# CognitiveAISystems/MAPF-GPT

Measured on AMD Instinct MI355X. Metric: agent-steps/s (env+obs+GPT fwd), higher is better.
Workload: dtype f16x3

## Files before the change

### mapf_gpt_amd/csrc/gpt_kernels_attn_tiles.h

```cpp
#pragma once
#include "gpt_kernels_c256p.h"

namespace mgpt {
namespace fastk {

constexpr int kAttNvb1 = 10, kAttNvb2 = 6;

__device__ unsigned long long g_attn_fallbacks = 0;

template <class T, int NP, int KROW, int VROW, int HS>
__device__ __forceinline__ void attention_exact_tiles(unsigned kr_addr, unsigned vr_addr, const u32x4 (&qf)[2][2], float sc2, f32x16 &o, float &l_run)
{
    float m_run, zero;
    asm volatile("v_mov_b32 %0, 0xff800000\n\tv_mov_b32 %1, 0" : "=v"(m_run), "=v"(zero));
    l_run = zero;
#pragma unroll
    for (int g = 0; g < 16; g++) o[g] = zero;
{
    u32x4 kf[2][2], vf[2][2];
    auto load_k = [&](int kt) {
        const unsigned a = kr_addr + (unsigned)kt * (32 * KROW);
        asm volatile("ds_read_b128 %0, %1" : "=v"(kf[0][0]) : "v"(a) : "memory");
        asm volatile("ds_read_b128 %0, %1 offset:32" : "=v"(kf[1][0]) : "v"(a) : "memory");
        if (NP == 2) {
            asm volatile("ds_read_b128 %0, %1 offset:%2" : "=v"(kf[0][1]) : "v"(a), "n"(kT * KROW) : "memory");
            asm volatile("ds_read_b128 %0, %1 offset:%2" : "=v"(kf[1][1]) : "v"(a), "n"(kT * KROW + 32) : "memory");
        } else { kf[0][1] = kf[0][0]; kf[1][1] = kf[1][0]; }
    };
    load_k(0);
#pragma unroll 1
    for (int kt = 0; kt < kT / 32; kt++) {
        f32x16 sc;
#pragma unroll
        for (int g = 0; g < 16; g++) sc[g] = 0.f;
        asm volatile("s_waitcnt lgkmcnt(0)" ::: "memory");
        __builtin_amdgcn_sched_barrier(0);
#pragma unroll
        for (int ks = 0; ks < 2; ks++) sc = mma<T, NP>(kf[ks], qf[ks], sc);
        __builtin_amdgcn_sched_barrier(0);
        {
            const unsigned a = vr_addr + (unsigned)kt * 64;
            asm volatile("ds_read_b128 %0, %1" : "=v"(vf[0][0]) : "v"(a) : "memory");
            asm volatile("ds_read_b128 %0, %1 offset:32" : "=v"(vf[1][0]) : "v"(a) : "memory");
            if (NP == 2) {
                asm volatile("ds_read_b128 %0, %1 offset:%2" : "=v"(vf[0][1]) : "v"(a), "n"(HS * VROW) : "memory");
                asm volatile("ds_read_b128 %0, %1 offset:%2" : "=v"(vf[1][1]) : "v"(a), "n"(HS * VROW + 32) : "memory");
            } else { vf[0][1] = vf[0][0]; vf[1][1] = vf[1][0]; }
        }
        if (kt + 1 < kT / 32) load_k(kt + 1);
        float mx = sc[0];
#pragma unroll
        for (int g = 1; g < 16; g++) mx = fmaxf(mx, sc[g]);
        mx = other_half_max(mx);
        if (__builtin_amdgcn_ballot_w64(mx > m_run) != 0) {
            const float m_new = fmaxf(m_run, mx);
            const float alpha = __builtin_amdgcn_exp2f((m_run - m_new) * sc2);
            l_run *= alpha;
#pragma unroll
            for (int g = 0; g < 16; g++) o[g] *= alpha;
            m_run = m_new;
        }
        const float nm = -m_run * sc2;
        float psum = 0.f;
#pragma unroll
        for (int g = 0; g < 16; g++) {
            sc[g] = __builtin_amdgcn_exp2f(fmaf(sc[g], sc2, nm));
            psum += sc[g];
        }
        l_run += other_half_sum(psum);
        u32x4 pf[2][2];
#pragma unroll
        for (int mm = 0; mm < 2; mm++) pack_octet<T, NP>(sc, mm, pf[mm]);
        if (kt + 1 < kT / 32) asm volatile("s_waitcnt lgkmcnt(%0)" ::"n"(2 * NP) : "memory");
        else asm volatile("s_waitcnt lgkmcnt(0)" ::: "memory");
        __builtin_amdgcn_sched_barrier(0);
#pragma unroll
        for (int mm = 0; mm < 2; mm++) o = mma<T, NP>(vf[mm], pf[mm], o);
    }
}
}

template <class T, int NP, int KROW, int VROW, int HS>
__device__ __forceinline__ void attention_tiles(unsigned kr_addr, unsigned vr_addr, const u32x4 (&qf)[2][2], int lane, f32x16 &o, float &l_run)
{
    using I0 = std::integral_constant<int, 0>;
    using I1 = std::integral_constant<int, 1>;

    u32x4 kf[2][2], vf[2][2], pf[2][2];
    f32x16 sA, sB;
    constexpr int NM = NP == 2 ? 3 : 1;
    auto amfma = [&](u32x4 a, u32x4 b2, f32x16 c) { return T::mfma(a, b2, c); };
    auto amma = [&](const u32x4 (&a)[2], const u32x4 (&b2)[2], f32x16 c) {
        if (NP == 2) { c = amfma(a[1], b2[0], c); c = amfma(a[0], b2[1], c); }
        return amfma(a[0], b2[0], c);
    };
    auto load_k = [&](auto kt_c) {
        constexpr int off = decltype(kt_c)::value * (32 * KROW);
        asm volatile("ds_read_b128 %0, %1 offset:%2" : "=v"(kf[0][0]) : "v"(kr_addr), "n"(off) : "memory");
        asm volatile("ds_read_b128 %0, %1 offset:%2" : "=v"(kf[1][0]) : "v"(kr_addr), "n"(off + 32) : "memory");
        if (NP == 2) {
            asm volatile("ds_read_b128 %0, %1 offset:%2" : "=v"(kf[0][1]) : "v"(kr_addr), "n"(off + kT * KROW) : "memory");
            asm volatile("ds_read_b128 %0, %1 offset:%2" : "=v"(kf[1][1]) : "v"(kr_addr), "n"(off + kT * KROW + 32) : "memory");
        } else { kf[0][1] = kf[0][0]; kf[1][1] = kf[1][0]; }
    };
    auto load_v = [&](auto kt_c, auto mm_c) {
        constexpr int off = decltype(kt_c)::value * 64 + decltype(mm_c)::value * 32, mm = decltype(mm_c)::value;
        asm volatile("ds_read_b128 %0, %1 offset:%2" : "=v"(vf[mm][0]) : "v"(vr_addr), "n"(off) : "memory");
        if (NP == 2) asm volatile("ds_read_b128 %0, %1 offset:%2" : "=v"(vf[mm][1]) : "v"(vr_addr), "n"(off + HS * VROW) : "memory");
        else vf[mm][1] = vf[mm][0];
    };
    auto lgkm = [&](auto n_c) {
        asm volatile("s_waitcnt lgkmcnt(%0)" ::"n"(decltype(n_c)::value) : "memory");
        __builtin_amdgcn_sched_barrier(0);
    };
    auto place = [&](auto nmf_c, auto nv_c) {
#pragma unroll
        for (int n = 0; n < decltype(nmf_c)::value; n++) {
            __builtin_amdgcn_sched_group_barrier(0x008, 1, 0);
            __builtin_amdgcn_sched_group_barrier(0x002, decltype(nv_c)::value, 0);
        }
        __builtin_amdgcn_sched_group_barrier(0x002, 64, 0);
        __builtin_amdgcn_sched_barrier(0);
    };
    using LK = std::integral_constant<int, 2 * NP>;
    using LV = std::integral_constant<int, NP>;
    load_k(I0{});
    lgkm(I0{});
#pragma unroll
    for (int g = 0; g < 16; g++) sA[g] = 0.f;
#pragma unroll
    for (int ks = 0; ks < 2; ks++) sA = amma(kf[ks], qf[ks], sA);
    __builtin_amdgcn_sched_barrier(0);
    load_k(I1{});
    f32x16 nmb;
    {
        float mx = sA[0];
#pragma unroll
        for (int g = 1; g < 16; g++) mx = fmaxf(mx, sA[g]);
        const float nm = -other_half_max(mx);
#pragma unroll
        for (int g = 0; g < 16; g++) { nmb[g] = nm; sA[g] += nm; }
    }
    float l_part = 0.f;
    auto tile = [&](auto kt_c, f32x16 &cur, f32x16 &nxt) {
        constexpr int kt = decltype(kt_c)::value;
        constexpr bool FIRSTT = kt == 0, LASTT = kt == kT / 32 - 1, HAS2 = kt + 2 < kT / 32;
        if constexpr (!FIRSTT) {
            lgkm(std::integral_constant<int, LASTT ? 0 : LK::value>{});
            o = amma(vf[1], pf[1], o);
#pragma unroll
            for (int g = 0; g < 4; g++) {
                cur[g] = __builtin_amdgcn_exp2f(cur[g]);
                l_part += cur[g];
            }
            place(std::integral_constant<int, NM>{}, std::integral_constant<int, 4>{});
            asm volatile("" : "+v"(o));
        }
        load_v(kt_c, I0{});
        if constexpr (!LASTT) {
            lgkm(LV{});
            nxt = amma(kf[0], qf[0], nmb);
            nxt = amma(kf[1], qf[1], nxt);
        }
#pragma unroll
        for (int g = FIRSTT ? 0 : 4; g < 16; g++) {
            cur[g] = __builtin_amdgcn_exp2f(cur[g]);
            l_part += cur[g];
        }
        pack_octet<T, NP>(cur, 0, pf[0]);
        place(std::integral_constant<int, LASTT ? 0 : 2 * NM>{}, std::integral_constant<int, kAttNvb1>{});
        if constexpr (!LASTT) asm volatile("" : "+v"(nxt));
        load_v(kt_c, I1{});
        lgkm(LV{});
        if constexpr (FIRSTT) {
#pragma unroll
            for (int g = 0; g < 16; g++) o[g] = 0.f;
        }
        o = amma(vf[0], pf[0], o);
        pack_octet<T, NP>(cur, 1, pf[1]);
        place(std::integral_constant<int, NM>{}, std::integral_constant<int, kAttNvb2>{});
        asm volatile("" : "+v"(o));
        if constexpr (HAS2) load_k(std::integral_constant<int, HAS2 ? kt + 2 : 0>{});
    };
    using K0 = std::integral_constant<int, 0>; using K1 = std::integral_constant<int, 1>; using K2 = std::integral_constant<int, 2>; using K3 = std::integral_constant<int, 3>;
    using K4 = std::integral_constant<int, 4>; using K5 = std::integral_constant<int, 5>; using K6 = std::integral_constant<int, 6>; using K7 = std::integral_constant<int, 7>;
    static_assert(kT / 32 == 8, "eight key tiles");
    tile(K0{}, sA, sB); tile(K1{}, sB, sA); tile(K2{}, sA, sB); tile(K3{}, sB, sA);
    tile(K4{}, sA, sB); tile(K5{}, sB, sA); tile(K6{}, sA, sB); tile(K7{}, sB, sA);
    lgkm(I0{});
    o = amma(vf[1], pf[1], o);
    __builtin_amdgcn_sched_barrier(0);
    l_run = other_half_sum(l_part);
    if (__builtin_amdgcn_ballot_w64(!(l_part < 60000.0f)) != 0) {
        if (lane == 0) atomicAdd(&g_attn_fallbacks, 1ull);
        attention_exact_tiles<T, NP, KROW, VROW, HS>(kr_addr, vr_addr, qf, 1.0f, o, l_run);
    }
}

}
}
```

### mapf_gpt_amd/csrc/gpt_kernels_c256b.h

```cpp
#pragma once
#include "gpt_kernels_c256p.h"
#include "gpt_kernels_attn_tiles.h"

namespace mgpt {
namespace fastk {

constexpr int kA256oProjSteps = 16;
constexpr int kA256oPeriod = 8 * kA256StepsPerHead + kA256oProjSteps;


template <class T, int NP>
__global__ __launch_bounds__(256) void pack_attn256q_kernel(const float *__restrict__ w_attn, const float *__restrict__ gain,
                                                            const float *__restrict__ w_proj, uint16_t *__restrict__ out,
                                                            float scale_a, float scale_p)
{
    constexpr int C = 256, NH = 8, QKV = NH * kA256StepsPerHead;
    const int64_t gid = (int64_t)blockIdx.x * 256 + threadIdx.x;
    if (gid >= (int64_t)kA256oPeriod * 8 * 64) return;
    const int lane = (int)(gid & 63), ms = (int)((gid >> 6) & 7), G = (int)(gid >> 9);
    const int rho = lane & 15, qk = lane >> 4;
    float v[8];
    if (G < QKV) {
        const int head = G / kA256StepsPerHead, st = G - head * kA256StepsPerHead;
        int which, kb, dim;
        if (st < 4) {
            const int cc = 4 * st + (ms >> 1), ug = ms & 1, rq = rho >> 2;
            kb = cc >> 1; which = cc & 1;
            const int blk = which == 0 ? 2 * (rq & 1) + (rq >> 1) : rq;
            dim = 8 * blk + 4 * ug + (rho & 3);
        } else { which = 2; kb = 4 * (st - 4) + (ms >> 1); dim = 16 * (ms & 1) + rho; }
        const float *row = w_attn + (size_t)(which * C + head * 32 + dim) * C;
#pragma unroll
        for (int e = 0; e < 8; e++) {
            const int col = 32 * kb + 8 * qk + e;
            v[e] = row[col] * gain[col] * scale_a;
        }
    } else {
        const int s = G - QKV, tt = s >> 2, j = s & 3;
        const int cc = 4 * j + (ms >> 1), kb = cc >> 1, fgl = 2 * (cc & 1) + (ms & 1);
        const float *row = w_proj + (size_t)(64 * tt + 16 * fgl + rho) * C;
#pragma unroll
        for (int e = 0; e < 8; e++) {
            const int col = 32 * kb + (e & 3) + 8 * (2 * (qk & 1) + (e >> 2)) + 4 * (qk >> 1);
            v[e] = row[col] * scale_p;
        }
    }
    u32x2 h0, l0, h1, l1;
    split4<T, NP>(v, h0, l0);
    split4<T, NP>(v + 4, h1, l1);
    u32x4 hi, lo;
    hi[0] = h0[0]; hi[1] = h0[1]; hi[2] = h1[0]; hi[3] = h1[1];
    lo[0] = l0[0]; lo[1] = l0[1]; lo[2] = l1[0]; lo[3] = l1[1];
    uint16_t *dst = out + (((size_t)G * 8 + ms) * NP) * 512 + (size_t)lane * 8;
    *reinterpret_cast<u32x4 *>(dst) = hi;
    if (NP == 2) *reinterpret_cast<u32x4 *>(dst + 512) = lo;
}

template <int NP> constexpr int kL0TabHeadBytes = 192 * NP;
template <int NP> constexpr int kL0TabEntryBytes = 8 * kL0TabHeadBytes<NP>;
template <class T, int NP, bool EMB = false, int TAB = 0>
__global__ __launch_bounds__(512, 2) void attn256q_kernel(float *__restrict__ x, const uint16_t *__restrict__ wstream, float inv_scale,
                                                          float scale_log2e, float inv_proj, unsigned char *__restrict__ spill,
                                                          int n_rows, const unsigned char *__restrict__ tokens = nullptr,
                                                          const float *__restrict__ etab = nullptr, unsigned char *__restrict__ table = nullptr)
{
    static_assert(TAB == 0 || (TAB == 1 && EMB) || (TAB == 2 && !EMB), "table modes");
    constexpr int HB = kL0TabHeadBytes<NP>, ENT = kL0TabEntryBytes<NP>;
    constexpr int C = 256, KS = 16, NH = 8, HS = 32, NW = 8;
    static_assert(NP == 2 || NP == 1, "planes");
    constexpr int MS = 8;
    constexpr int STEP = MS * NP * 1024;
    constexpr int NSLOT = 5;
    constexpr int PW = MS * NP / NW;
    constexpr int KROW = 80, VROW = 528;
    constexpr int NSPILL = 2 * NP;
    constexpr int NYLD = 14 * NP;
    static_assert(PW >= 1, "a wave moves at least one piece per step");
    extern __shared__ __attribute__((aligned(16))) unsigned char smem[];
    const int tid = threadIdx.x, lane = tid & 63;
    const int wave = __builtin_amdgcn_readfirstlane(tid >> 6);
    const int tok0 = wave * 32;
    const unsigned lane16 = (unsigned)lane * 16u;
    const unsigned lds0 = (unsigned)(size_t)smem + lane16;
    const unsigned sK = (unsigned)(size_t)smem + NSLOT * STEP, sV = sK + NP * kT * KROW;
    constexpr int PERIOD = TAB == 2 ? kA256oProjSteps : kA256oPeriod;
    const unsigned char *wbase = reinterpret_cast<const unsigned char *>(wstream) + (size_t)(wave * PW) * 1024 +
                                 (TAB == 2 ? (size_t)(kA256oPeriod - kA256oProjSteps) * STEP : 0);
    unsigned char *sp_wave = spill + ((size_t)blockIdx.x * NW + wave) * (size_t)(14 * NP * 1024);
    const int n_mine = n_rows > (int)blockIdx.x ? (n_rows - 1 - (int)blockIdx.x) / (int)gridDim.x + 1 : 0;
    if (n_mine == 0) return;

    int r_issue = 0;
    int slot_cur = 0, slot_prev = NSLOT - 1;
    unsigned cur_addr = 0, nxt_addr = 0;
    auto issue = [&](int slot) {
        const unsigned char *src = wbase + (size_t)r_issue * STEP;
        unsigned char *dst = smem + (size_t)slot * STEP + (size_t)(wave * PW) * 1024;
#pragma unroll
        for (int i = 0; i < PW; i++) dma_piece(src + lane16, dst, std::integral_constant<int, 0>{}, i);
        r_issue = r_issue + 1 == PERIOD ? 0 : r_issue + 1;
    };
#pragma unroll
    for (int G = 0; G < NSLOT - 1; G++) issue(G);
    auto sync_wait = [&](auto pending_c) {
        vm_wait<decltype(pending_c)::value>();
        __builtin_amdgcn_s_barrier();
    };
    int slot_refill = 0;
    auto sync_issue = [&]() {
        issue(slot_prev);
        const int slot_next = slot_cur + 1 == NSLOT ? 0 : slot_cur + 1;
        cur_addr = lds0 + (unsigned)slot_cur * STEP;
        nxt_addr = lds0 + (unsigned)slot_next * STEP;
        slot_prev = slot_cur;
        slot_cur = slot_next;
    };
    u32x4 wb[2][2][2];
    auto chunk_wait = [&]() {
        asm volatile("s_waitcnt lgkmcnt(0)" ::: "memory");
        __builtin_amdgcn_sched_barrier(0);
    };
    auto chunk_read = [&](auto c_c, auto next_c, auto n_c) {
        constexpr int c = decltype(c_c)::value, n = decltype(n_c)::value;
        if constexpr (n < 2 * NP) {
            constexpr int fr = n / NP, pl = n % NP;
            if constexpr (c < 3) lds_frag(cur_addr, std::integral_constant<int, ((2 * c + 2 + fr) * NP + pl) * 1024>{}, wb[(c + 1) & 1][fr][pl]);
            else if constexpr (decltype(next_c)::value) lds_frag(nxt_addr, std::integral_constant<int, (fr * NP + pl) * 1024>{}, wb[0][fr][pl]);
            if constexpr (NP == 1 && (c < 3 || decltype(next_c)::value)) wb[(c + 1) & 1][fr][1] = wb[(c + 1) & 1][fr][0];
            __builtin_amdgcn_sched_barrier(0);
        }
    };
    using I0 = std::integral_constant<int, 0>;
    using I1 = std::integral_constant<int, 1>;
    using I2 = std::integral_constant<int, 2>;
    using I3 = std::integral_constant<int, 3>;
    auto mma4 = [&](const u32x4 (&w0)[2], const u32x4 (&w1)[2], const u32x4 (&x0)[2], const u32x4 (&x1)[2], f32x16 &blk, auto swap_c, auto first_c, auto &&behind) {
        constexpr bool SW = decltype(swap_c)::value, FIRST = decltype(first_c)::value;
        auto one = [&](const u32x4 &w, const u32x4 &xx, auto s_c) {
            if constexpr (SW) mm16<T>(xx, w, blk, s_c); else mm16<T>(w, xx, blk, s_c);
        };
        auto onez = [&](const u32x4 &w, const u32x4 &xx, auto s_c) {
            if constexpr (!FIRST) one(w, xx, s_c);
            else if constexpr (SW) mm16z<T>(xx, w, blk, s_c);
            else mm16z<T>(w, xx, blk, s_c);
        };
        if (NP == 2) {
            onez(w0[1], x0[0], I0{}); behind(I0{}); onez(w1[1], x0[0], I1{}); behind(I1{}); onez(w0[1], x1[0], I2{}); behind(I2{}); onez(w1[1], x1[0], I3{}); behind(I3{});
            one(w0[0], x0[1], I0{}); behind(std::integral_constant<int, 4>{}); one(w1[0], x0[1], I1{}); behind(std::integral_constant<int, 5>{});
            one(w0[0], x1[1], I2{}); one(w1[0], x1[1], I3{});
            one(w0[0], x0[0], I0{}); one(w1[0], x0[0], I1{}); one(w0[0], x1[0], I2{}); one(w1[0], x1[0], I3{});
        } else {
            onez(w0[0], x0[0], I0{}); behind(I0{}); onez(w1[0], x0[0], I1{}); behind(I1{}); onez(w0[0], x1[0], I2{}); behind(I2{}); onez(w1[0], x1[0], I3{});
        }
    };
    auto chunk_body = [&](auto c_c, auto next_c, auto &&mm) {
        chunk_wait();
        constexpr bool REFILL = false;
        constexpr int N_REFILL = NP == 2 ? 5 : 2, N_LAST = REFILL ? N_REFILL : 2 * NP - 1, NMF = NP == 2 ? 12 : 4;
        mm([&](auto n_c) {
            constexpr int n = decltype(n_c)::value;
            if constexpr (n < 2 * NP) { __builtin_amdgcn_sched_barrier(0); chunk_read(c_c, next_c, n_c); }
            else if constexpr (REFILL && n == N_REFILL) { __builtin_amdgcn_sched_barrier(0); issue(slot_refill); __builtin_amdgcn_sched_barrier(0); }
        });
#pragma unroll
        for (int n = 0; n < NMF - 1 - N_LAST; n++) __builtin_amdgcn_sched_group_barrier(0x008, 1, 0);
        __builtin_amdgcn_sched_barrier(0);
    };
    const float q_units = scale_log2e * inv_scale, k_units = inv_scale;

    u32x4 xn[KS][2];

    f32x16 qa, ka;
    auto step_pair = [&](auto j_c, auto pending_c, auto &&after_barrier, auto next_c) {
        constexpr int j = decltype(j_c)::value;
        sync_wait(pending_c);
        after_barrier();
        sync_issue();
        auto chunk = [&](auto c_c) {
            constexpr int c = decltype(c_c)::value;
            constexpr int cc = 4 * j + c, kb = cc >> 1;
            chunk_body(c_c, next_c, [&](auto &&behind) {
                using F = std::integral_constant<bool, (cc < 2)>;
                if constexpr ((cc & 1) == 0) mma4(wb[c & 1][0], wb[c & 1][1], xn[kb], xn[8 + kb], qa, std::false_type{}, F{}, behind);
                else mma4(wb[c & 1][0], wb[c & 1][1], xn[kb], xn[8 + kb], ka, std::false_type{}, F{}, behind);
            });
            asm volatile("" : "+v"(qa), "+v"(ka));
        };
        chunk(I0{}); chunk(I1{}); chunk(I2{}); chunk(I3{});
    };
    auto nothing = [&]() {};
    asm volatile("s_waitcnt vmcnt(0)" ::: "memory");
    __builtin_amdgcn_s_barrier();
    nxt_addr = lds0;
    using P4 = std::integral_constant<int, PW * (NSLOT - 3)>;
    using P4S = std::integral_constant<int, PW * (NSLOT - 3) + NSPILL>;

#pragma unroll 1
    for (int k = 0; k < n_mine; k++) {
        const int64_t b = (int64_t)blockIdx.x + (int64_t)k * gridDim.x;
        unsigned char *xw = reinterpret_cast<unsigned char *>(x + (b * kT + tok0) * C);
        unsigned ent0 = 0, ent1 = 0;
        if constexpr (TAB == 2) {
            unsigned l16p = lane16;
            asm volatile("" : "+v"(l16p));
            const unsigned char *tk = tokens + b * kT + tok0;
            const unsigned tt_p = (l16p >> 4) & 15u;
            unsigned id0, id1;
            asm volatile("global_load_ubyte %0, %1, %2" : "=v"(id0) : "v"(tt_p), "s"(tk) : "memory");
            asm volatile("global_load_ubyte %0, %1, %2 offset:16" : "=v"(id1) : "v"(tt_p), "s"(tk) : "memory");
            asm volatile("s_waitcnt vmcnt(0)" : "+v"(id0), "+v"(id1) : : "memory");
            ent0 = ((unsigned)tok0 + tt_p) * 67u + id0;
            ent1 = ((unsigned)tok0 + 16u + tt_p) * 67u + id1;
        } else {
            unsigned l16p = lane16;
            asm volatile("" : "+v"(l16p));
            const unsigned xoff_p = (l16p >> 8) * 1024 + ((l16p >> 4) & 15u) * 32;
            f32x4 xr[32];
            if constexpr (EMB) {
                const unsigned char *tk = tokens + b * kT + tok0;
                const unsigned tt_p = (l16p >> 4) & 15u;
                unsigned id0, id1;
                asm volatile("global_load_ubyte %0, %1, %2" : "=v"(id0) : "v"(tt_p), "s"(tk) : "memory");
                asm volatile("global_load_ubyte %0, %1, %2 offset:16" : "=v"(id1) : "v"(tt_p), "s"(tk) : "memory");
                asm volatile("s_waitcnt vmcnt(0)" : "+v"(id0), "+v"(id1) : : "memory");
                const unsigned q32 = (l16p >> 8) * 32u;
                const unsigned ve0 = (((unsigned)tok0 + tt_p) * 67u + id0) * 1024u + q32;
                const unsigned ve1 = (((unsigned)tok0 + 16u + tt_p) * 67u + id1) * 1024u + q32;
                const unsigned char *eb = reinterpret_cast<const unsigned char *>(etab);
#pragma unroll
                for (int i = 0; i < 32; i++) {
                    if (((i >> 1) & 1) == 0)
                        asm volatile("global_load_dwordx4 %0, %1, %2 offset:%3" : "=v"(xr[2 * (i >> 2) + (i & 1)]) : "v"(ve0), "s"(eb), "n"((i >> 2) * 128 + (i & 1) * 16) : "memory");
                    else
                        asm volatile("global_load_dwordx4 %0, %1, %2 offset:%3" : "=v"(xr[2 * (8 + (i >> 2)) + (i & 1)]) : "v"(ve1), "s"(eb), "n"((i >> 2) * 128 + (i & 1) * 16) : "memory");
                }
            } else {
#pragma unroll
            for (int i = 0; i < 32; i++) {
                const unsigned char *xq = xw + (i >> 2) * 4096;
                asm volatile("global_load_dwordx4 %0, %1, %2 offset:%3" : "=v"(xr[2 * (8 * ((i >> 1) & 1) + (i >> 2)) + (i & 1)]) : "v"(xoff_p), "s"(xq), "n"(((i >> 1) & 1) * 512 + (i & 1) * 16) : "memory");
            }
            }
            asm volatile("s_waitcnt vmcnt(0)" : "+v"(xr[0]), "+v"(xr[1]), "+v"(xr[2]), "+v"(xr[3]), "+v"(xr[4]), "+v"(xr[5]), "+v"(xr[6]), "+v"(xr[7]) : : "memory");
            asm volatile("" : "+v"(xr[8]), "+v"(xr[9]), "+v"(xr[10]), "+v"(xr[11]), "+v"(xr[12]), "+v"(xr[13]), "+v"(xr[14]), "+v"(xr[15]));
            asm volatile("" : "+v"(xr[16]), "+v"(xr[17]), "+v"(xr[18]), "+v"(xr[19]), "+v"(xr[20]), "+v"(xr[21]), "+v"(xr[22]), "+v"(xr[23]));
            asm volatile("" : "+v"(xr[24]), "+v"(xr[25]), "+v"(xr[26]), "+v"(xr[27]), "+v"(xr[28]), "+v"(xr[29]), "+v"(xr[30]), "+v"(xr[31]));
            if constexpr (EMB) {
#pragma unroll
                for (int i = 0; i < 32; i++) {
                    const unsigned char *xq = xw + (i >> 2) * 4096;
                    asm volatile("global_store_dwordx4 %0, %1, %2 offset:%3\n\ts_nop 1" ::"v"(xoff_p), "v"(xr[2 * (8 * ((i >> 1) & 1) + (i >> 2)) + (i & 1)]), "s"(xq), "n"(((i >> 1) & 1) * 512 + (i & 1) * 16) : "memory");
                }
            }
            float rstd[2];
#pragma unroll
            for (int tg = 0; tg < 2; tg++) {
                float sm = 0.f;
#pragma unroll
                for (int i = 0; i < 16; i++) sm += (xr[16 * tg + i][0] + xr[16 * tg + i][1]) + (xr[16 * tg + i][2] + xr[16 * tg + i][3]);
                const float mean = permlane_fold4(sm) * (1.0f / (float)C);
                float qv = 0.f;
#pragma unroll
                for (int i = 0; i < 16; i++)
#pragma unroll
                    for (int e = 0; e < 4; e++) { const float d = xr[16 * tg + i][e] - mean; xr[16 * tg + i][e] = d; qv = fmaf(d, d, qv); }
                rstd[tg] = rsqrtf(permlane_fold4(qv) * (1.0f / (float)C) + 1e-5f);
            }
#pragma unroll
            for (int ks = 0; ks < KS; ks++) {
                float v0[4], v1[4];
#pragma unroll
                for (int e = 0; e < 4; e++) { v0[e] = xr[2 * ks][e] * rstd[ks >> 3]; v1[e] = xr[2 * ks + 1][e] * rstd[ks >> 3]; }
                u32x2 h0, l0, h1, l1;
                split4p<T, NP>(v0, h0, l0);
                split4p<T, NP>(v1, h1, l1);
                xn[ks][0][0] = h0[0]; xn[ks][0][1] = h0[1]; xn[ks][0][2] = h1[0]; xn[ks][0][3] = h1[1];
                xn[ks][1][0] = l0[0]; xn[ks][1][1] = l0[1]; xn[ks][1][2] = l1[0]; xn[ks][1][3] = l1[1];
                if ((ks & 1) == 1) __builtin_amdgcn_sched_barrier(0);
            }
        }
        if constexpr (TAB != 2) {
            lds_pair<NP>(nxt_addr, I0{}, wb[0][0]);
            lds_pair<NP>(nxt_addr, I1{}, wb[0][1]);
        }

        auto head = [&](int hd, auto last_c) {
            constexpr bool LASTH = decltype(last_c)::value;
            unsigned l16 = lane16;
            asm volatile("" : "+v"(l16));
            const unsigned rr = (l16 >> 4) & 31u, hh = l16 >> 9;
            const unsigned kr_addr = sK + rr * KROW + hh * 16;
            const unsigned vr_addr = sV + rr * VROW + hh * 16;
            const unsigned tt = (l16 >> 4) & 15u, qq = l16 >> 8;
            const unsigned kw_addr = sK + ((unsigned)tok0 + tt) * KROW + qq * 16;
            const unsigned vw_addr = sV + tt * VROW + (unsigned)wave * 64 + (qq & 1u) * 16 + (qq >> 1) * 8;
            asm volatile("" : "=v"(qa), "=v"(ka));
            step_pair(I0{}, P4S{}, nothing, std::true_type{});
            step_pair(I1{}, P4S{}, nothing, std::true_type{});
            step_pair(I2{}, P4S{}, nothing, std::true_type{});
            step_pair(I3{}, P4{}, nothing, std::true_type{});
            u32x4 qf[2][2];
#pragma unroll
            for (int g = 0; g < 16; g++) { qa[g] *= q_units; ka[g] *= k_units; }
#pragma unroll
            for (int tg = 0; tg < 2; tg++) pack_octet<T, NP>(qa, tg, qf[tg]);
#pragma unroll
            for (int pl = 0; pl < NP; pl++)
#pragma unroll
                for (int wd = 0; wd < 4; wd++) { unsigned a = qf[0][pl][wd], b2 = qf[1][pl][wd]; row_swap(a, b2); qf[0][pl][wd] = a; qf[1][pl][wd] = b2; }
            if (NP == 1) { qf[0][1] = qf[0][0]; qf[1][1] = qf[1][0]; }
            if constexpr (TAB == 1) {
                const unsigned voff = (((unsigned)tok0 + rr) * 67u * ENT) + (unsigned)b * ENT + (unsigned)hd * HB + hh * (32 * NP);
#pragma unroll
                for (int ks = 0; ks < 2; ks++)
#pragma unroll
                    for (int pl = 0; pl < NP; pl++)
                        asm volatile("global_store_dwordx4 %0, %1, %2 offset:%3\n\ts_nop 1" ::"v"(voff), "v"(qf[ks][pl]), "s"(table), "n"((ks * NP + pl) * 16) : "memory");
            }
            {
                u32x4 kp[2][2];
#pragma unroll
                for (int tg = 0; tg < 2; tg++) pack_octet<T, NP>(ka, tg, kp[tg]);
#pragma unroll
                for (int tg = 0; tg < 2; tg++)
#pragma unroll
                    for (int pl = 0; pl < NP; pl++)
                        asm volatile("ds_write_b128 %0, %1 offset:%2" ::"v"(kw_addr), "v"(kp[tg][pl]), "n"(pl * kT * KROW + tg * 16 * KROW) : "memory");
                if constexpr (TAB == 1) {
#pragma unroll
                    for (int tg = 0; tg < 2; tg++) {
                        const unsigned voff = (((unsigned)tok0 + 16u * tg + tt) * 67u * ENT) + (unsigned)b * ENT + (unsigned)hd * HB + 64 * NP + qq * (16 * NP);
#pragma unroll
                        for (int pl = 0; pl < NP; pl++)
                            asm volatile("global_store_dwordx4 %0, %1, %2 offset:%3\n\ts_nop 1" ::"v"(voff), "v"(kp[tg][pl]), "s"(table), "n"(pl * 16) : "memory");
                    }
                }
            }
            f32x16 va;
            auto step_v = [&](auto j_c, auto next_c) {
                constexpr int j = decltype(j_c)::value;
                sync_wait(P4{});
                sync_issue();
                auto chunk = [&](auto c_c) {
                    constexpr int c = decltype(c_c)::value;
                    constexpr int kb = 4 * j + c;
                    chunk_body(c_c, next_c, [&](auto &&behind) { mma4(wb[c & 1][0], wb[c & 1][1], xn[kb], xn[8 + kb], va, std::true_type{}, std::integral_constant<bool, kb == 0>{}, behind); });
                    asm volatile("" : "+v"(va));
                };
                chunk(I0{}); chunk(I1{}); chunk(I2{}); chunk(I3{});
            };
            step_v(I0{}, std::true_type{});
            step_v(I1{}, std::false_type{});
            if constexpr (LASTH) {
#pragma unroll
                for (int hh2 = 0; hh2 < 7; hh2++)
#pragma unroll
                    for (int tg = 0; tg < 2; tg++)
#pragma unroll
                        for (int pl = 0; pl < NP; pl++) {
                            const unsigned char *p = sp_wave + (size_t)hh2 * (size_t)(2 * NP * 1024);
                            asm volatile("global_load_dwordx4 %0, %1, %2 offset:%3" : "=v"(xn[8 * tg + hh2][pl]) : "v"(lane16), "s"(p), "n"((tg * NP + pl) * 1024) : "memory");
                        }
            }
            {
#pragma unroll
                for (int sl = 0; sl < 4; sl++) {
                    u32x2 vp[2];
                    unsigned a0, b0, a1, b1;
                    split2p<T, NP>(va[4 * sl], va[4 * sl + 1], a0, b0);
                    split2p<T, NP>(va[4 * sl + 2], va[4 * sl + 3], a1, b1);
                    vp[0][0] = a0; vp[0][1] = a1; vp[1][0] = b0; vp[1][1] = b1;
#pragma unroll
                    for (int pl = 0; pl < NP; pl++)
                        asm volatile("ds_write_b64 %0, %1 offset:%2" ::"v"(vw_addr), "v"(vp[pl]), "n"(pl * HS * VROW + (sl & 1) * 16 * VROW + (sl >> 1) * 32) : "memory");
                    if constexpr (TAB == 1) {
#pragma unroll
                        for (int i = 0; i < 4; i++) {
                            const unsigned voff = (((unsigned)tok0 + 16u * (sl >> 1) + 4u * qq + i) * 67u * ENT) + (unsigned)b * ENT + (unsigned)hd * HB + 128 * NP +
                                                  (16u * (sl & 1) + tt) * 2u;
#pragma unroll
                            for (int pl = 0; pl < NP; pl++) {
                                if (i & 1) asm volatile("global_store_short_d16_hi %0, %1, %2 offset:%3" ::"v"(voff), "v"(vp[pl][i >> 1]), "s"(table), "n"(pl * 64) : "memory");
                                else asm volatile("global_store_short %0, %1, %2 offset:%3" ::"v"(voff), "v"(vp[pl][i >> 1]), "s"(table), "n"(pl * 64) : "memory");
                            }
                        }
                    }
                }
            }
            if constexpr (TAB == 1) asm volatile("s_waitcnt vmcnt(0)" ::: "memory");
            asm volatile("s_waitcnt lgkmcnt(0)" ::: "memory");
            __builtin_amdgcn_s_barrier();

            f32x16 o;
            float l_run = 0.f;
            attention_tiles<T, NP, KROW, VROW, HS>(kr_addr, vr_addr, qf, lane, o, l_run);
            lds_pair<NP>(nxt_addr, I0{}, wb[0][0]);
            lds_pair<NP>(nxt_addr, I1{}, wb[0][1]);
            {
                const float inv = inv_scale / l_run;
#pragma unroll
                for (int g = 0; g < 16; g++) o[g] *= inv;
#pragma unroll
                for (int g = 0; g < 8; g++) { float a = o[g], b2 = o[8 + g]; asm volatile("s_nop 1\n\tv_permlane16_swap_b32 %0, %1" : "+v"(a), "+v"(b2)); o[g] = a; o[8 + g] = b2; }
                if constexpr (LASTH) {
                    pack_octet<T, NP>(o, 0, xn[7]);
                    pack_octet<T, NP>(o, 1, xn[15]);
                } else {
                    u32x4 yp[2][2];
                    pack_octet<T, NP>(o, 0, yp[0]);
                    pack_octet<T, NP>(o, 1, yp[1]);
                    unsigned char *p = sp_wave + (size_t)hd * (size_t)(2 * NP * 1024);
#pragma unroll
                    for (int kk = 0; kk < 2; kk++)
#pragma unroll
                        for (int pl = 0; pl < NP; pl++)
                            asm volatile("global_store_dwordx4 %0, %1, %2 offset:%3\n\ts_nop 1" ::"v"(lane16), "v"(yp[kk][pl]), "s"(p), "n"((kk * NP + pl) * 1024) : "memory");
                }
            }
        };
        auto head_t = [&](int hd) {
            unsigned l16 = lane16;
            asm volatile("" : "+v"(l16));
            const unsigned rr = (l16 >> 4) & 31u, hh = l16 >> 9;
            const unsigned kr_addr = sK + rr * KROW + hh * 16;
            const unsigned vr_addr = sV + rr * VROW + hh * 16;
            const unsigned tt = (l16 >> 4) & 15u, qq = l16 >> 8;
            const unsigned kw_addr = sK + ((unsigned)tok0 + tt) * KROW + qq * 16;
            const unsigned vt_addr = sV + qq * 8 * VROW + (unsigned)wave * 64 + (((tt >> 2) & 1u) * 8 + ((tt >> 3) & 1u) * 4 + (tt & 3u)) * 2;
            const unsigned hoff = (unsigned)hd * HB;
            const unsigned e0 = ent0 * ENT + hoff, e1 = ent1 * ENT + hoff;
            const unsigned qoff = ((qq & 1u) ? e1 : e0) + hh * (32 * NP);
            u32x4 qf[2][2], kp[2][2], vq[2][2];
#pragma unroll
            for (int ks = 0; ks < 2; ks++)
#pragma unroll
                for (int pl = 0; pl < NP; pl++)
                    asm volatile("global_load_dwordx4 %0, %1, %2 offset:%3" : "=v"(qf[ks][pl]) : "v"(qoff), "s"(table), "n"((ks * NP + pl) * 16) : "memory");
#pragma unroll
            for (int tg = 0; tg < 2; tg++) {
                const unsigned ko = (tg ? e1 : e0) + qq * (16 * NP), vo = (tg ? e1 : e0) + qq * 16;
#pragma unroll
                for (int pl = 0; pl < NP; pl++) {
                    asm volatile("global_load_dwordx4 %0, %1, %2 offset:%3" : "=v"(kp[tg][pl]) : "v"(ko), "s"(table), "n"(64 * NP + pl * 16) : "memory");
                    asm volatile("global_load_dwordx4 %0, %1, %2 offset:%3" : "=v"(vq[tg][pl]) : "v"(vo), "s"(table), "n"(128 * NP + pl * 64) : "memory");
                }
            }
            __builtin_amdgcn_s_barrier();
            if constexpr (NP == 2)
                asm volatile("s_waitcnt vmcnt(0)" : "+v"(qf[0][0]), "+v"(qf[0][1]), "+v"(qf[1][0]), "+v"(qf[1][1]), "+v"(kp[0][0]), "+v"(kp[0][1]), "+v"(kp[1][0]), "+v"(kp[1][1]),
                             "+v"(vq[0][0]), "+v"(vq[0][1]), "+v"(vq[1][0]), "+v"(vq[1][1]) : : "memory");
            else
                asm volatile("s_waitcnt vmcnt(0)" : "+v"(qf[0][0]), "+v"(qf[1][0]), "+v"(kp[0][0]), "+v"(kp[1][0]), "+v"(vq[0][0]), "+v"(vq[1][0]) : : "memory");
            if (NP == 1) { qf[0][1] = qf[0][0]; qf[1][1] = qf[1][0]; }
#pragma unroll
            for (int tg = 0; tg < 2; tg++)
#pragma unroll
                for (int pl = 0; pl < NP; pl++) {
                    asm volatile("ds_write_b128 %0, %1 offset:%2" ::"v"(kw_addr), "v"(kp[tg][pl]), "n"(pl * kT * KROW + tg * 16 * KROW) : "memory");
#pragma unroll
                    for (int j = 0; j < 8; j++) {
                        if (j & 1) asm volatile("ds_write_b16_d16_hi %0, %1 offset:%2" ::"v"(vt_addr), "v"(vq[tg][pl][j >> 1]), "n"(pl * HS * VROW + j * VROW + tg * 32) : "memory");
                        else asm volatile("ds_write_b16 %0, %1 offset:%2" ::"v"(vt_addr), "v"(vq[tg][pl][j >> 1]), "n"(pl * HS * VROW + j * VROW + tg * 32) : "memory");
                    }
                }
            asm volatile("s_waitcnt lgkmcnt(0)" ::: "memory");
            __builtin_amdgcn_s_barrier();
            f32x16 o;
            float l_run = 0.f;
            attention_tiles<T, NP, KROW, VROW, HS>(kr_addr, vr_addr, qf, lane, o, l_run);
            const float inv = inv_scale / l_run;
#pragma unroll
            for (int g = 0; g < 16; g++) o[g] *= inv;
#pragma unroll
            for (int g = 0; g < 8; g++) { float a = o[g], b2 = o[8 + g]; asm volatile("s_nop 1\n\tv_permlane16_swap_b32 %0, %1" : "+v"(a), "+v"(b2)); o[g] = a; o[8 + g] = b2; }
#pragma unroll
            for (int k2 = 0; k2 < 7; k2++)
#pragma unroll
                for (int pl = 0; pl < NP; pl++) { xn[k2][pl] = xn[k2 + 1][pl]; xn[8 + k2][pl] = xn[9 + k2][pl]; }
            pack_octet<T, NP>(o, 0, xn[7]);
            pack_octet<T, NP>(o, 1, xn[15]);
        };
        if constexpr (TAB == 2) {
#pragma unroll 1
            for (int hd = 0; hd < NH; hd++) head_t(hd);
            lds_pair<NP>(nxt_addr, I0{}, wb[0][0]);
            lds_pair<NP>(nxt_addr, I1{}, wb[0][1]);
        } else {
#pragma unroll 1
            for (int hd = 0; hd < NH - 1; hd++) head(hd, std::false_type{});
            head(NH - 1, std::true_type{});
        }

        auto tail = [&](int t, auto first_c, auto last_c) {
            constexpr bool FIRST = decltype(first_c)::value, LASTT = decltype(last_c)::value;
            asm volatile("" : "=v"(qa), "=v"(ka));
            unsigned l16t = lane16;
            asm volatile("" : "+v"(l16t));
            const unsigned xoff_t = (l16t >> 9) * 1024 + ((l16t >> 4) & 15u) * 32 + ((l16t >> 8) & 1u) * 16;
            const unsigned qq_t = l16t >> 8;
            f32x4 xs[4][2];
            unsigned char *xp = xw + (size_t)t * 8192;
            constexpr int OTHERS = 8;
            auto requests = [&]() {
                if constexpr (TAB == 2) {
                    const unsigned r0 = ent0 * (C * 4) + (unsigned)t * 256 + qq_t * 16, r1 = ent1 * (C * 4) + (unsigned)t * 256 + qq_t * 16;
                    const unsigned char *eb = reinterpret_cast<const unsigned char *>(etab);
#pragma unroll
                    for (int fgl = 0; fgl < 4; fgl++) {
                        asm volatile("global_load_dwordx4 %0, %1, %2 offset:%3" : "=v"(xs[fgl][0]) : "v"(r0), "s"(eb), "n"(fgl * 64) : "memory");
                        asm volatile("global_load_dwordx4 %0, %1, %2 offset:%3" : "=v"(xs[fgl][1]) : "v"(r1), "s"(eb), "n"(fgl * 64) : "memory");
                    }
                    return;
                }
#pragma unroll
                for (int fgl = 0; fgl < 4; fgl++)
#pragma unroll
                    for (int tg = 0; tg < 2; tg++)
                        asm volatile("global_load_dwordx4 %0, %1, %2 offset:%3" : "=v"(xs[fgl][tg]) : "v"(xoff_t), "s"(xp + (fgl >> 1) * 4096), "n"((fgl & 1) * 2048 + tg * 512) : "memory");
            };
            step_pair(I0{}, std::integral_constant<int, 2 * PW + (FIRST ? (TAB == 2 ? 0 : NYLD) : 8)>{}, requests, std::true_type{});
            step_pair(I1{}, std::integral_constant<int, 2 * PW + 8 + OTHERS>{}, nothing, std::true_type{});
            step_pair(I2{}, std::integral_constant<int, 2 * PW + 8 + OTHERS>{}, nothing, std::true_type{});
            step_pair(I3{}, P4{}, nothing, std::integral_constant<bool, !LASTT>{});
            asm volatile("s_waitcnt vmcnt(%[n])" : "+v"(xs[0][0]), "+v"(xs[0][1]), "+v"(xs[1][0]), "+v"(xs[1][1]), "+v"(xs[2][0]), "+v"(xs[2][1]), "+v"(xs[3][0]), "+v"(xs[3][1])
                         : [n] "n"(4 * PW) : "memory");
#pragma unroll
            for (int fgl = 0; fgl < 4; fgl++)
#pragma unroll
                for (int tg = 0; tg < 2; tg++) {
                    f32x4 v;
#pragma unroll
                    for (int e = 0; e < 4; e++) v[e] = fmaf((fgl < 2 ? qa : ka)[4 * (2 * tg + (fgl & 1)) + e], inv_proj, xs[fgl][tg][e]);
                    asm volatile("global_store_dwordx4 %0, %1, %2 offset:%3\n\ts_nop 1" ::"v"(xoff_t), "v"(v), "s"(xp + (fgl >> 1) * 4096), "n"((fgl & 1) * 2048 + tg * 512) : "memory");
                }
        };
        {
            asm volatile("s_waitcnt vmcnt(0)" : "+v"(xn[0][0]), "+v"(xn[0][1]), "+v"(xn[1][0]), "+v"(xn[1][1]), "+v"(xn[2][0]), "+v"(xn[2][1]), "+v"(xn[3][0]), "+v"(xn[3][1]),
                         "+v"(xn[4][0]), "+v"(xn[4][1]), "+v"(xn[5][0]), "+v"(xn[5][1]), "+v"(xn[6][0]), "+v"(xn[6][1]) : : "memory");
            asm volatile("" : "+v"(xn[8][0]), "+v"(xn[8][1]), "+v"(xn[9][0]), "+v"(xn[9][1]), "+v"(xn[10][0]), "+v"(xn[10][1]), "+v"(xn[11][0]), "+v"(xn[11][1]),
                         "+v"(xn[12][0]), "+v"(xn[12][1]), "+v"(xn[13][0]), "+v"(xn[13][1]), "+v"(xn[14][0]), "+v"(xn[14][1]));
            asm volatile("" : "+v"(xn[7][0]), "+v"(xn[7][1]), "+v"(xn[15][0]), "+v"(xn[15][1]));
        }
        tail(0, std::true_type{}, std::false_type{});
#pragma unroll 1
        for (int t = 1; t < 3; t++) tail(t, std::false_type{}, std::false_type{});
        tail(3, std::false_type{}, std::true_type{});
    }
    asm volatile("s_waitcnt vmcnt(0)" ::: "memory");
}

}
}
```

Before: 128,300.

## Prefetch next head's Q/K/V table rows during attention via hook and LDS staging

In the TAB==2 path, the next head's K/V table entries are now staged into LDS with global_load_lds right after each head's barrier. The next head's Q fragments are prefetched into registers through a new hook called inside attention_tiles near the final tile. A fallback hook reloads the current Q if the exact-attention path runs. The weight-ring DMA prologue is deferred until the last head and held during the last tail step, with the vmcnt waits adjusted to match. The aim is to hide global-load latency of per-head table reads behind attention compute, at the cost of more complex wait-count bookkeeping and extra LDS staging space.

After: 128,300 (median of 3 runs). No clear change (-0.0%).

```diff
diff --git a/mapf_gpt_amd/csrc/gpt_kernels_attn_tiles.h b/mapf_gpt_amd/csrc/gpt_kernels_attn_tiles.h
--- a/mapf_gpt_amd/csrc/gpt_kernels_attn_tiles.h
+++ b/mapf_gpt_amd/csrc/gpt_kernels_attn_tiles.h
@@ -80,8 +80,12 @@
 }
 }
 
-template <class T, int NP, int KROW, int VROW, int HS>
-__device__ __forceinline__ void attention_tiles(unsigned kr_addr, unsigned vr_addr, const u32x4 (&qf)[2][2], int lane, f32x16 &o, float &l_run)
+struct attn_no_hook {
+    template <class P> __device__ __forceinline__ void operator()(P) const {}
+};
+
+template <class T, int NP, int KROW, int VROW, int HS, class Hook = attn_no_hook>
+__device__ __forceinline__ void attention_tiles(unsigned kr_addr, unsigned vr_addr, const u32x4 (&qf)[2][2], int lane, f32x16 &o, float &l_run, Hook hook = Hook{})
 {
     using I0 = std::integral_constant<int, 0>;
     using I1 = std::integral_constant<int, 1>;
@@ -170,6 +174,7 @@
         pack_octet<T, NP>(cur, 0, pf[0]);
         place(std::integral_constant<int, LASTT ? 0 : 2 * NM>{}, std::integral_constant<int, kAttNvb1>{});
         if constexpr (!LASTT) asm volatile("" : "+v"(nxt));
+        if constexpr (kt == kT / 32 - 2) hook(I0{});
         load_v(kt_c, I1{});
         lgkm(LV{});
         if constexpr (FIRSTT) {
@@ -193,7 +198,9 @@
     l_run = other_half_sum(l_part);
     if (__builtin_amdgcn_ballot_w64(!(l_part < 60000.0f)) != 0) {
         if (lane == 0) atomicAdd(&g_attn_fallbacks, 1ull);
+        hook(I1{});
         attention_exact_tiles<T, NP, KROW, VROW, HS>(kr_addr, vr_addr, qf, 1.0f, o, l_run);
+        hook(std::integral_constant<int, 2>{});
     }
 }
 
diff --git a/mapf_gpt_amd/csrc/gpt_kernels_c256b.h b/mapf_gpt_amd/csrc/gpt_kernels_c256b.h
--- a/mapf_gpt_amd/csrc/gpt_kernels_c256b.h
+++ b/mapf_gpt_amd/csrc/gpt_kernels_c256b.h
@@ -93,15 +93,19 @@
     int r_issue = 0;
     int slot_cur = 0, slot_prev = NSLOT - 1;
     unsigned cur_addr = 0, nxt_addr = 0;
+    bool ring_hold = false;
     auto issue = [&](int slot) {
+        if constexpr (TAB == 2) { if (ring_hold) return; }
         const unsigned char *src = wbase + (size_t)r_issue * STEP;
         unsigned char *dst = smem + (size_t)slot * STEP + (size_t)(wave * PW) * 1024;
 #pragma unroll
         for (int i = 0; i < PW; i++) dma_piece(src + lane16, dst, std::integral_constant<int, 0>{}, i);
         r_issue = r_issue + 1 == PERIOD ? 0 : r_issue + 1;
     };
+    if constexpr (TAB != 2) {
 #pragma unroll
     for (int G = 0; G < NSLOT - 1; G++) issue(G);
+    }
     auto sync_wait = [&](auto pending_c) {
         vm_wait<decltype(pending_c)::value>();
         __builtin_amdgcn_s_barrier();
@@ -211,6 +215,7 @@
             asm volatile("s_waitcnt vmcnt(0)" : "+v"(id0), "+v"(id1) : : "memory");
             ent0 = ((unsigned)tok0 + tt_p) * 67u + id0;
             ent1 = ((unsigned)tok0 + 16u + tt_p) * 67u + id1;
+            asm volatile("" : "+v"(ent0), "+v"(ent1));
         } else {
             unsigned l16p = lane16;
             asm volatile("" : "+v"(l16p));
@@ -418,6 +423,7 @@
                 }
             }
         };
+        u32x4 qf[2][2];
         auto head_t = [&](int hd) {
             unsigned l16 = lane16;
             asm volatile("" : "+v"(l16));
@@ -428,29 +434,49 @@
             const unsigned kw_addr = sK + ((unsigned)tok0 + tt) * KROW + qq * 16;
             const unsigned vt_addr = sV + qq * 8 * VROW + (unsigned)wave * 64 + (((tt >> 2) & 1u) * 8 + ((tt >> 3) & 1u) * 4 + (tt & 3u)) * 2;
             const unsigned hoff = (unsigned)hd * HB;
-            const unsigned e0 = ent0 * ENT + hoff, e1 = ent1 * ENT + hoff;
+            unsigned en0 = ent0, en1 = ent1;
+            asm volatile("" : "+v"(en0), "+v"(en1));
+            const unsigned e0 = en0 * ENT + hoff, e1 = en1 * ENT + hoff;
             const unsigned qoff = ((qq & 1u) ? e1 : e0) + hh * (32 * NP);
-            u32x4 qf[2][2], kp[2][2], vq[2][2];
-#pragma unroll
-            for (int ks = 0; ks < 2; ks++)
-#pragma unroll
-                for (int pl = 0; pl < NP; pl++)
-                    asm volatile("global_load_dwordx4 %0, %1, %2 offset:%3" : "=v"(qf[ks][pl]) : "v"(qoff), "s"(table), "n"((ks * NP + pl) * 16) : "memory");
-#pragma unroll
-            for (int tg = 0; tg < 2; tg++) {
-                const unsigned ko = (tg ? e1 : e0) + qq * (16 * NP), vo = (tg ? e1 : e0) + qq * 16;
-#pragma unroll
-                for (int pl = 0; pl < NP; pl++) {
-                    asm volatile("global_load_dwordx4 %0, %1, %2 offset:%3" : "=v"(kp[tg][pl]) : "v"(ko), "s"(table), "n"(64 * NP + pl * 16) : "memory");
-                    asm volatile("global_load_dwordx4 %0, %1, %2 offset:%3" : "=v"(vq[tg][pl]) : "v"(vo), "s"(table), "n"(128 * NP + pl * 64) : "memory");
-                }
-            }
-            __builtin_amdgcn_s_barrier();
-            if constexpr (NP == 2)
-                asm volatile("s_waitcnt vmcnt(0)" : "+v"(qf[0][0]), "+v"(qf[0][1]), "+v"(qf[1][0]), "+v"(qf[1][1]), "+v"(kp[0][0]), "+v"(kp[0][1]), "+v"(kp[1][0]), "+v"(kp[1][1]),
-                             "+v"(vq[0][0]), "+v"(vq[0][1]), "+v"(vq[1][0]), "+v"(vq[1][1]) : : "memory");
-            else
-                asm volatile("s_waitcnt vmcnt(0)" : "+v"(qf[0][0]), "+v"(qf[1][0]), "+v"(kp[0][0]), "+v"(kp[1][0]), "+v"(vq[0][0]), "+v"(vq[1][0]) : : "memory");
+            u32x4 kp[2][2], vq[2][2];
+            const unsigned st_addr = (unsigned)(size_t)smem + l16 + (unsigned)wave * (4 * NP * 1024);
+            if (hd == 0) {
+#pragma unroll
+                for (int ks = 0; ks < 2; ks++)
+#pragma unroll
+                    for (int pl = 0; pl < NP; pl++)
+                        asm volatile("global_load_dwordx4 %0, %1, %2 offset:%3" : "=v"(qf[ks][pl]) : "v"(qoff), "s"(table), "n"((ks * NP + pl) * 16) : "memory");
+#pragma unroll
+                for (int tg = 0; tg < 2; tg++) {
+                    const unsigned ko = (tg ? e1 : e0) + qq * (16 * NP), vo = (tg ? e1 : e0) + qq * 16;
+#pragma unroll
+                    for (int pl = 0; pl < NP; pl++) {
+                        asm volatile("global_load_dwordx4 %0, %1, %2 offset:%3" : "=v"(kp[tg][pl]) : "v"(ko), "s"(table), "n"(64 * NP + pl * 16) : "memory");
+                        asm volatile("global_load_dwordx4 %0, %1, %2 offset:%3" : "=v"(vq[tg][pl]) : "v"(vo), "s"(table), "n"(128 * NP + pl * 64) : "memory");
+                    }
+                }
+                __builtin_amdgcn_s_barrier();
+                if constexpr (NP == 2)
+                    asm volatile("s_waitcnt vmcnt(0)" : "+v"(qf[0][0]), "+v"(qf[0][1]), "+v"(qf[1][0]), "+v"(qf[1][1]), "+v"(kp[0][0]), "+v"(kp[0][1]), "+v"(kp[1][0]), "+v"(kp[1][1]),
+                                 "+v"(vq[0][0]), "+v"(vq[0][1]), "+v"(vq[1][0]), "+v"(vq[1][1]) : : "memory");
+                else
+                    asm volatile("s_waitcnt vmcnt(0)" : "+v"(qf[0][0]), "+v"(qf[1][0]), "+v"(kp[0][0]), "+v"(kp[1][0]), "+v"(vq[0][0]), "+v"(vq[1][0]) : : "memory");
+            } else {
+                __builtin_amdgcn_s_barrier();
+                if constexpr (NP == 2) asm volatile("s_waitcnt vmcnt(0)" : "+v"(qf[0][0]), "+v"(qf[0][1]), "+v"(qf[1][0]), "+v"(qf[1][1]) : : "memory");
+                else asm volatile("s_waitcnt vmcnt(0)" : "+v"(qf[0][0]), "+v"(qf[1][0]) : : "memory");
+#pragma unroll
+                for (int tg = 0; tg < 2; tg++)
+#pragma unroll
+                    for (int pl = 0; pl < NP; pl++) {
+                        asm volatile("ds_read_b128 %0, %1 offset:%2" : "=v"(kp[tg][pl]) : "v"(st_addr), "n"(2 * (tg * NP + pl) * 1024) : "memory");
+                        asm volatile("ds_read_b128 %0, %1 offset:%2" : "=v"(vq[tg][pl]) : "v"(st_addr), "n"((2 * (tg * NP + pl) + 1) * 1024) : "memory");
+                    }
+                if constexpr (NP == 2)
+                    asm volatile("s_waitcnt lgkmcnt(0)" : "+v"(kp[0][0]), "+v"(kp[0][1]), "+v"(kp[1][0]), "+v"(kp[1][1]), "+v"(vq[0][0]), "+v"(vq[0][1]), "+v"(vq[1][0]), "+v"(vq[1][1]) : : "memory");
+                else
+                    asm volatile("s_waitcnt lgkmcnt(0)" : "+v"(kp[0][0]), "+v"(kp[1][0]), "+v"(vq[0][0]), "+v"(vq[1][0]) : : "memory");
+            }
             if (NP == 1) { qf[0][1] = qf[0][0]; qf[1][1] = qf[1][0]; }
 #pragma unroll
             for (int tg = 0; tg < 2; tg++)
@@ -465,9 +491,47 @@
                 }
             asm volatile("s_waitcnt lgkmcnt(0)" ::: "memory");
             __builtin_amdgcn_s_barrier();
+            if (hd < NH - 1) {
+                unsigned char *stg = smem + (size_t)wave * (size_t)(4 * NP * 1024);
+                const unsigned char *tb = table + HB;
+#pragma unroll
+                for (int tg = 0; tg < 2; tg++) {
+                    const unsigned ko = (tg ? e1 : e0) + qq * (16 * NP), vo = (tg ? e1 : e0) + qq * 16;
+#pragma unroll
+                    for (int pl = 0; pl < NP; pl++) {
+                        __builtin_amdgcn_global_load_lds((gbl_void_t *)(tb + ko + (64 * NP + pl * 16)), (lds_void_t *)(stg + 2 * (tg * NP + pl) * 1024), 16, 0, 0);
+                        __builtin_amdgcn_global_load_lds((gbl_void_t *)(tb + vo + (128 * NP + pl * 64)), (lds_void_t *)(stg + (2 * (tg * NP + pl) + 1) * 1024), 16, 0, 0);
+                    }
+                }
+            } else {
+                int s_p = slot_cur;
+#pragma unroll
+                for (int G = 0; G < NSLOT - 1; G++) { issue(s_p); s_p = s_p + 1 == NSLOT ? 0 : s_p + 1; }
+            }
+            const unsigned qnext = qoff + (hd < NH - 1 ? (unsigned)HB : 0u);
+            auto q_hook = [&](auto p_c) {
+                constexpr int P = decltype(p_c)::value;
+                if constexpr (P == 1) {
+                    const unsigned qthis = qnext - (hd < NH - 1 ? (unsigned)HB : 0u);
+#pragma unroll
+                    for (int ks = 0; ks < 2; ks++)
+#pragma unroll
+                        for (int pl = 0; pl < NP; pl++)
+                            asm volatile("global_load_dwordx4 %0, %1, %2 offset:%3" : "=v"(qf[ks][pl]) : "v"(qthis), "s"(table), "n"((ks * NP + pl) * 16) : "memory");
+                    if constexpr (NP == 2) asm volatile("s_waitcnt vmcnt(0)" : "+v"(qf[0][0]), "+v"(qf[0][1]), "+v"(qf[1][0]), "+v"(qf[1][1]) : : "memory");
+                    else asm volatile("s_waitcnt vmcnt(0)" : "+v"(qf[0][0]), "+v"(qf[1][0]) : : "memory");
+                    if (NP == 1) { qf[0][1] = qf[0][0]; qf[1][1] = qf[1][0]; }
+                } else {
+#pragma unroll
+                    for (int ks = 0; ks < 2; ks++)
+#pragma unroll
+                        for (int pl = 0; pl < NP; pl++)
+                            asm volatile("global_load_dwordx4 %0, %1, %2 offset:%3" : "=v"(qf[ks][pl]) : "v"(qnext), "s"(table), "n"((ks * NP + pl) * 16) : "memory");
+                }
+            };
             f32x16 o;
             float l_run = 0.f;
-            attention_tiles<T, NP, KROW, VROW, HS>(kr_addr, vr_addr, qf, lane, o, l_run);
+            attention_tiles<T, NP, KROW, VROW, HS>(kr_addr, vr_addr, qf, lane, o, l_run, q_hook);
             const float inv = inv_scale / l_run;
 #pragma unroll
             for (int g = 0; g < 16; g++) o[g] *= inv;
@@ -483,8 +547,6 @@
         if constexpr (TAB == 2) {
 #pragma unroll 1
             for (int hd = 0; hd < NH; hd++) head_t(hd);
-            lds_pair<NP>(nxt_addr, I0{}, wb[0][0]);
-            lds_pair<NP>(nxt_addr, I1{}, wb[0][1]);
         } else {
 #pragma unroll 1
             for (int hd = 0; hd < NH - 1; hd++) head(hd, std::false_type{});
@@ -510,6 +572,10 @@
                         asm volatile("global_load_dwordx4 %0, %1, %2 offset:%3" : "=v"(xs[fgl][0]) : "v"(r0), "s"(eb), "n"(fgl * 64) : "memory");
                         asm volatile("global_load_dwordx4 %0, %1, %2 offset:%3" : "=v"(xs[fgl][1]) : "v"(r1), "s"(eb), "n"(fgl * 64) : "memory");
                     }
+                    if constexpr (FIRST) {
+                        lds_pair<NP>(nxt_addr, I0{}, wb[0][0]);
+                        lds_pair<NP>(nxt_addr, I1{}, wb[0][1]);
+                    }
                     return;
                 }
 #pragma unroll
@@ -518,12 +584,15 @@
                     for (int tg = 0; tg < 2; tg++)
                         asm volatile("global_load_dwordx4 %0, %1, %2 offset:%3" : "=v"(xs[fgl][tg]) : "v"(xoff_t), "s"(xp + (fgl >> 1) * 4096), "n"((fgl & 1) * 2048 + tg * 512) : "memory");
             };
+            constexpr bool HOLD = TAB == 2 && LASTT;
+            if constexpr (HOLD) ring_hold = true;
             step_pair(I0{}, std::integral_constant<int, 2 * PW + (FIRST ? (TAB == 2 ? 0 : NYLD) : 8)>{}, requests, std::true_type{});
-            step_pair(I1{}, std::integral_constant<int, 2 * PW + 8 + OTHERS>{}, nothing, std::true_type{});
-            step_pair(I2{}, std::integral_constant<int, 2 * PW + 8 + OTHERS>{}, nothing, std::true_type{});
-            step_pair(I3{}, P4{}, nothing, std::integral_constant<bool, !LASTT>{});
+            step_pair(I1{}, std::integral_constant<int, (HOLD ? PW : 2 * PW) + 8 + OTHERS>{}, nothing, std::true_type{});
+            step_pair(I2{}, std::integral_constant<int, (HOLD ? 0 : 2 * PW) + 8 + OTHERS>{}, nothing, std::true_type{});
+            step_pair(I3{}, std::integral_constant<int, HOLD ? OTHERS : P4::value>{}, nothing, std::integral_constant<bool, !LASTT>{});
+            if constexpr (HOLD) ring_hold = false;
             asm volatile("s_waitcnt vmcnt(%[n])" : "+v"(xs[0][0]), "+v"(xs[0][1]), "+v"(xs[1][0]), "+v"(xs[1][1]), "+v"(xs[2][0]), "+v"(xs[2][1]), "+v"(xs[3][0]), "+v"(xs[3][1])
-                         : [n] "n"(4 * PW) : "memory");
+                         : [n] "n"(HOLD ? 0 : 4 * PW) : "memory");
 #pragma unroll
             for (int fgl = 0; fgl < 4; fgl++)
 #pragma unroll
@@ -540,6 +609,7 @@
             asm volatile("" : "+v"(xn[8][0]), "+v"(xn[8][1]), "+v"(xn[9][0]), "+v"(xn[9][1]), "+v"(xn[10][0]), "+v"(xn[10][1]), "+v"(xn[11][0]), "+v"(xn[11][1]),
                          "+v"(xn[12][0]), "+v"(xn[12][1]), "+v"(xn[13][0]), "+v"(xn[13][1]), "+v"(xn[14][0]), "+v"(xn[14][1]));
             asm volatile("" : "+v"(xn[7][0]), "+v"(xn[7][1]), "+v"(xn[15][0]), "+v"(xn[15][1]));
+            if constexpr (TAB == 2) asm volatile("" : "+v"(qf[0][0]), "+v"(qf[0][1]), "+v"(qf[1][0]), "+v"(qf[1][1]));
         }
         tail(0, std::true_type{}, std::false_type{});
 #pragma unroll 1
```
